# avabag01-ai/spectrogram-midi

Hardware: AMD Instinct MI355X
Metric: audio-seconds transcribed/sec (44.1 kHz, n_fft=2048) (higher is better)
Workload: dtype f64

## Files before the change

### spectrogram-midi_amd/csrc/aegis_handle.hip

```cpp
#include "aegis_internal.h"
#include "effects.h"

#include <chrono>
#include <cmath>
#include <cstdio>
#include <cstdlib>
#include <new>
#include <stdexcept>
#include <thread>

using namespace aegis;

static std::string g_create_error;

int aegis::grow_buf(aegis_handle *h, std::vector<DevBuf *> &owner, DevBuf &b, size_t bytes) {
    if (h->fail_allocs > 0) {
        --h->fail_allocs;
        h->err = "hipMalloc(" + std::to_string(bytes) + " bytes): out of memory (test hook)";
        return AEGIS_ERR_NOMEM;
    }
    if (b.p) {
        HIPCHK(h, hipDeviceSynchronize());
        HIPCHK(h, hipFree(b.p));
        b.p = nullptr; b.cap = 0;
    }
    if (!b.listed) { owner.push_back(&b); b.listed = true; }
    const size_t want = bytes + bytes / 8 + 256;
    hipError_t e = hipMalloc(&b.p, want);
    if (e != hipSuccess) {
        b.p = nullptr;
        h->err = "hipMalloc(" + std::to_string(want) + " bytes): " + hipGetErrorString(e);
        return AEGIS_ERR_NOMEM;
    }
    b.cap = want;
    return AEGIS_OK;
}

void aegis::free_bufs(std::vector<DevBuf *> &owner) noexcept {
    for (DevBuf *b : owner) {
        if (b->p) (void)hipFree(b->p);
        *b = DevBuf{};
    }
    owner.clear();
}

int aegis::new_event(aegis_handle *h, hipEvent_t *e, unsigned flags) {
    HIPCHK(h, hipEventCreateWithFlags(e, flags));
    h->owned_events.push_back(*e);
    return AEGIS_OK;
}

static int create_events(aegis_handle *h) {
    int rc = new_event(h, &h->copy_event, hipEventDisableTiming);
    h->sync_events.assign(8, nullptr);
    for (hipEvent_t &e : h->sync_events) if (rc == AEGIS_OK) rc = new_event(h, &e, hipEventDisableTiming);
    for (hipEvent_t &e : h->split_ev) if (rc == AEGIS_OK) rc = new_event(h, &e, hipEventDefault);
    for (hipEvent_t &e : h->hyb_ev) if (rc == AEGIS_OK) rc = new_event(h, &e, hipEventDisableTiming);
    for (hipEvent_t &e : h->fin_ev) if (rc == AEGIS_OK) rc = new_event(h, &e, hipEventDisableTiming);
    return rc;
}

template <typename T>
static int upload_table(aegis_handle *h, const std::vector<T> &v, const T **dst) {
    void *d = nullptr;
    const size_t bytes = std::max<size_t>(v.size() * sizeof(T), 16);
    HIPCHK(h, hipMalloc(&d, bytes));
    h->table_allocs.push_back(d);
    if (!v.empty()) HIPCHK(h, hipMemcpy(d, v.data(), v.size() * sizeof(T), hipMemcpyHostToDevice));
    *dst = static_cast<const T *>(d);
    return AEGIS_OK;
}

void aegis::begin_event(aegis_handle *h, const char *name, hipStream_t s) {
    if (!h->profiling) return;
    hipEvent_t a, b;
    if (hipEventCreate(&a) != hipSuccess || hipEventCreate(&b) != hipSuccess) return;
    (void)hipEventRecord(a, s);
    h->events.push_back({name, {a, b}});
}
void aegis::end_event(aegis_handle *h, hipStream_t s) {
    if (!h->profiling || h->events.empty()) return;
    (void)hipEventRecord(h->events.back().second.second, s);
}
void aegis::drop_events(aegis_handle *h) noexcept {
    for (auto &ev : h->events) { (void)hipEventDestroy(ev.second.first); (void)hipEventDestroy(ev.second.second); }
    h->events.clear();
}
void aegis::collect_events(aegis_handle *h) {
    h->last_ms.clear();
    h->last_count.clear();
    double total = 0;
    for (auto &ev : h->events) {
        float ms = 0;
        if (hipEventElapsedTime(&ms, ev.second.first, ev.second.second) == hipSuccess) {
            h->last_ms[ev.first] += ms;
            h->last_count[ev.first] += 1;
            total += ms;
        }
    }
    drop_events(h);
    h->last_ms["total"] = total;
}

int aegis::abi_fail(aegis_handle *h) noexcept {
    int code = AEGIS_ERR_DEVICE;
    const char *msg = "unknown C++ exception";
    std::string what;
    try { throw; }
    catch (const std::bad_alloc &) { code = AEGIS_ERR_NOMEM; msg = "out of host memory"; }
    catch (const std::length_error &) { code = AEGIS_ERR_NOMEM; msg = "request too large for a host container"; }
    catch (const std::exception &e) { try { what = e.what(); msg = what.c_str(); } catch (...) {} }
    catch (...) {}
    try { (h ? h->err : g_create_error) = msg; } catch (...) {}
    return code;
}

static const PassPlan *last_pass(const aegis_handle *h) { return h->plan.passes.empty() ? nullptr : &h->plan.passes.back(); }
static int last_work(const aegis_handle *h) { return h->plan.passes.empty() ? 0 : (int)((h->plan.passes.size() - 1) & 1); }

extern "C" {

int aegis_abi_version(void) { return AEGIS_ABI_VERSION; }

const char *aegis_last_error(const aegis_handle *h) { return h ? h->err.c_str() : g_create_error.c_str(); }

int aegis_create(const aegis_config *cfg, aegis_handle **out) {
    aegis_handle *h = nullptr;
    try {
    if (!out) { g_create_error = "out == NULL"; return AEGIS_ERR_INVALID; }
    *out = nullptr;
    aegis_config c{};
    if (cfg) c = *cfg;
    if (c.sample_rate == 0) c.sample_rate = 44100;
    if (c.hop_length == 0) c.hop_length = 512;
    if (c.n_fft == 0) c.n_fft = 2048;
    if (c.n_mels == 0) c.n_mels = 128;
    if (!(c.fmin > 0)) c.fmin = 82.4068892282175;
    if (!(c.fmax > 0)) c.fmax = 1046.5022612023945;
    const bool auto_pass = c.max_frames_per_pass <= 0;
    if (auto_pass) c.max_frames_per_pass = (int64_t)1 << 21;

    h = new (std::nothrow) aegis_handle();
    if (!h) { g_create_error = "out of host memory"; return AEGIS_ERR_NOMEM; }
    const std::string terr = h->tab.build(c.sample_rate, c.hop_length, c.n_fft, c.n_mels, c.fmin, c.fmax);
    if (!terr.empty()) { g_create_error = terr; delete h; return AEGIS_ERR_INVALID; }
    if (!h->tab.set_pyin_init(c.pyin_init)) { g_create_error = "pyin_init must be AEGIS_PYIN_INIT_UNVOICED (0) or AEGIS_PYIN_INIT_UNIFORM (1)"; delete h; return AEGIS_ERR_INVALID; }
    h->device = c.device;
    h->max_frames_per_pass = c.max_frames_per_pass;
    h->knobs.read_env();
    h->persist.on = h->knobs.persistent_wanted;

    h->lag_stride = (h->tab.max_period + 1 + 7) & ~7;
// ... 104 lines not shown
            bool busy = false;
            for (hipStream_t q : all) if (q && hipStreamQuery(q) == hipErrorNotReady) busy = true;
            if (!busy) break;
            if (std::chrono::steady_clock::now() - t0 > std::chrono::seconds(10)) {
                std::fprintf(stderr, "libaegis_hip: aegis_destroy: work still running on the handle's streams after 10 s; its device memory and streams are leaked\n");
                (void)hipGetLastError();
                delete h;
                return;
            }
            std::this_thread::sleep_for(std::chrono::milliseconds(1));
        }
        (void)hipGetLastError();
    }
    T("device sync");
    (void)hipDeviceSynchronize();
    for (auto &ss : h->split)
        for (hipStream_t q : {ss.frame_a, ss.frame_b, ss.viterbi})
            if (q) { T("destroy masked stream"); (void)hipStreamDestroy(q); }
    T("sync stream"); if (h->stream) (void)hipStreamSynchronize(h->stream);
    T("sync stream2"); if (h->stream2) (void)hipStreamSynchronize(h->stream2);
    T("sync stream3"); if (h->stream3) (void)hipStreamSynchronize(h->stream3);
    T("sync stream4"); if (h->stream4) (void)hipStreamSynchronize(h->stream4);
    T("events");
    drop_events(h);
    for (hipEvent_t e : h->owned_events) (void)hipEventDestroy(e);
    T("free tables");
    for (void *p : h->table_allocs) (void)hipFree(p);
    for (auto &cb : h->cqt_banks) if (cb.bank.dev) (void)hipFree(cb.bank.dev);
    h->cqt_banks.clear();
    T("free workspaces and staging");
    free_bufs(h->bufs);
    T("destroy streams");
    for (hipStream_t q : {h->stream, h->stream2, h->stream3, h->stream4}) if (q) (void)hipStreamDestroy(q);
    T("done");
    delete h;
}

extern "C" {

int64_t aegis_frames_for(const aegis_handle *h, int64_t n_samples) {
    try {
    if (!h || n_samples < 0) return AEGIS_ERR_INVALID;
    return 1 + n_samples / h->tab.hop;
    } catch (...) { return abi_fail(const_cast<aegis_handle *>(h)); }
}

int aegis_set_profiling(aegis_handle *h, int32_t on) {
    try {
    if (!h) return AEGIS_ERR_INVALID;
    h->profiling = on != 0;
    return AEGIS_OK;
    } catch (...) { return abi_fail(h); }
}

int aegis_last_kernel_launches(const aegis_handle *h, const char *name) {
    if (!h || !name) return -1;
    auto it = h->last_count.find(name);
    return it == h->last_count.end() ? 0 : it->second;
}

double aegis_last_kernel_ms(const aegis_handle *h, const char *name) {
    if (!h || !name) return -1.0;
    auto it = h->last_ms.find(name);
    return it == h->last_ms.end() ? -1.0 : it->second;
}

int aegis_set_table(aegis_handle *h, const char *name, const double *data, int64_t count) {
    try {
    if (!h || !name || !data) return AEGIS_ERR_INVALID;
    Tables &t = h->tab;
    const std::string n(name);
    struct Slot { std::vector<double> *host; const double *dev; };
    auto slot = [&](const std::string &nm) -> Slot {
        if (nm == "beta_probs") return {&t.beta_probs, h->dt.beta_probs};
        if (nm == "beta_cumsum") return {&t.beta_cumsum, h->dt.beta_cumsum};
        if (nm == "beta_suffix") return {&t.beta_suffix, h->dt.beta_suffix};
        if (nm == "boltz_fact") return {&t.boltz_fact, h->dt.boltz_fact};
        if (nm == "boltz_exp") return {&t.boltz_exp, h->dt.boltz_exp};
        if (nm == "freqs") return {&t.freqs, h->dt.freqs};
        return {nullptr, nullptr};
    };
    auto push = [&](const std::string &nm) -> int {
        Slot s = slot(nm);
        if (h->device < 0) return AEGIS_OK;
        HIPCHK(h, hipSetDevice(h->device));
        HIPCHK(h, hipStreamSynchronize(h->stream));
        HIPCHK(h, hipMemcpy(const_cast<double *>(s.dev), s.host->data(), s.host->size() * 8, hipMemcpyHostToDevice));
        return AEGIS_OK;
    };
    Slot s = slot(n);
    if (!s.host || n == "beta_cumsum" || n == "beta_suffix") { h->err = "unknown or derived table: " + n; return AEGIS_ERR_INVALID; }
    if (count != (int64_t)s.host->size()) {
        h->err = "table " + n + " needs " + std::to_string(s.host->size()) + " entries";
        return AEGIS_ERR_INVALID;
    }
    std::copy(data, data + count, s.host->begin());
    int rc = push(n);
    if (rc != AEGIS_OK) return rc;
    if (n == "beta_probs") {
        for (int k = 0; k <= kNThresholds; ++k) t.beta_cumsum[k] = np_pairwise_sum(t.beta_probs.data(), k);
        t.beta_suffix.assign(kNThresholds + 1, 0.0);
        for (int k = kNThresholds - 1; k >= 0; --k) t.beta_suffix[k] = t.beta_suffix[k + 1] + t.beta_probs[k];
        if ((rc = push("beta_cumsum")) != AEGIS_OK) return rc;
        if ((rc = push("beta_suffix")) != AEGIS_OK) return rc;
    }
    return AEGIS_OK;
    } catch (...) { return abi_fail(h); }
}

int64_t aegis_get_param(const aegis_handle *h, const char *name) {
    try {
    if (!h || !name) return AEGIS_ERR_INVALID;
    const Tables &t = h->tab;
    const std::string n(name);
    if (n == "min_period") return t.min_period;
    if (n == "max_period") return t.max_period;
    if (n == "n_lags") return t.n_lags;
    if (n == "n_pitch_bins") return t.n_bins;
    if (n == "transition_width") return t.width;
    if (n == "n_trans_classes") return t.n_cls;
    if (n == "max_frames_per_pass") return h->max_frames_per_pass;
    if (n == "lag_stride") return h->lag_stride;
    if (n == "yin_stride") return h->yin_stride;
    if (n == "obs_stride") return h->obs_stride;
    const PassPlan *lp = last_pass(h);
    if (n == "last_frames") return lp ? lp->fp : 0;
    if (n == "last_passes") return (int64_t)h->plan.passes.size();
    if (n == "last_split_segments") { int64_t v = 0; for (const PassPlan &q : h->plan.passes) v += q.tsplit ? q.n_seg : 0; return v; }
    if (n == "split_passes") return h->tsplit.stats[0];
    if (n == "split_segments") return h->tsplit.stats[1];
    if (n == "split_flagged_clips") return h->tsplit.stats[2];
    if (n == "split_unlocked_clips") return h->tsplit.stats[3];
    if (n == "split_rounds") return h->tsplit.last_carried_steps;
    if (n == "split_viterbi_us") return (int64_t)(h->tsplit.last_viterbi_ms * 1e3);
    if (n == "split_cooldown") return h->tsplit.cooldown;
    if (n == "last_chunks") return lp ? lp->nk() : 0;
    if (n == "last_dense") return lp ? lp->dense : 0;
    if (n == "last_proportional") return lp ? lp->proportional : 0;
    if (n == "last_balanced") return lp ? lp->balanced : 0;
    if (n == "last_hybrid_step") return lp ? lp->hyb_S : 0;
    if (n == "last_persistent") return lp ? lp->persistent : 0;
    if (n == "pyin_init") return t.pyin_init;
    if (n == "cqt_bank_builds") return h->cqt_bank_builds;
    if (n == "cqt_banks") return (int64_t)h->cqt_banks.size();
    if (n == "cqt_bank_cap") return h->cqt_bank_cap;
    if (n == "cqt_bank_bytes") return h->cqt_bank_bytes;
    if (n == "cqt_bank_build_us") return h->cqt_bank_build_us;
    if (n == "cmnd_in_frame") return cmnd_in_frame(h);
    if (n == "troughs_in_frame") return troughs_in_frame(h);
    if (n == "frame_fpw") return frame_batch_fpw(t.max_period);
    if (n == "obs_waves") { PassParams q = base_params(t); q.n_sel = 4096; return pyin_obs_waves(q); }
    if (n == "viterbi_kernel") { const int k = viterbi_kernel_choice(base_params(t), rule_tables(h)); return k < 0 ? AEGIS_ERR_UNSUPPORTED : k; }
    if (n == "split_applies") return viterbi_split_applies(base_params(t), rule_tables(h)) ? 1 : 0;
    if (n == "fx_tile") return kFxRevTile;
    if (n == "fx_chunk") return kFxChunk;
    if (n == "fx_max_taps") return kFxMaxTaps;
    return AEGIS_ERR_INVALID;
    } catch (...) { return abi_fail(const_cast<aegis_handle *>(h)); }
}

int64_t aegis_get_table(const aegis_handle *h, const char *name, void *dst, int64_t cap) {
    try {
    if (!h || !name) return AEGIS_ERR_INVALID;
    const Tables &t = h->tab;
    const std::string n(name);
    const void *src = nullptr;
    int64_t count = 0;
    size_t esz = 8;
    auto setd = [&](const std::vector<double> &v) { src = v.data(); count = (int64_t)v.size(); esz = 8; };
    if (n == "hann") setd(t.hann);
    else if (n == "thresholds") setd(t.thresholds);
    else if (n == "beta_probs") setd(t.beta_probs);
    else if (n == "beta_cumsum") setd(t.beta_cumsum);
    else if (n == "beta_suffix") setd(t.beta_suffix);
    else if (n == "boltz_fact") setd(t.boltz_fact);
    else if (n == "boltz_exp") setd(t.boltz_exp);
    else if (n == "log_trans_band") setd(t.log_trans_band);
    else if (n == "log_trans_pack") setd(t.log_trans_pack);
    else if (n == "freqs") setd(t.freqs);
    else if (n == "bin_edges") setd(t.bin_edges);
    else if (n == "twiddle") setd(t.twiddle);
    else if (n == "tuning_edges") setd(h->tuning_edges);
    else if (n == "mel_dense") { src = t.mel_dense.data(); count = (int64_t)t.mel_dense.size(); esz = 4; }
    else return AEGIS_ERR_INVALID;
    if (dst && cap > 0) std::memcpy(dst, src, (size_t)std::min(count, cap) * esz);
    return count;
    } catch (...) { return abi_fail(const_cast<aegis_handle *>(h)); }
}

int64_t aegis_debug_plan(aegis_handle *h, const int64_t *n_samples, int32_t n_clips, int32_t entry, int32_t sync,
                         int32_t n_cus, int64_t *dst, int64_t cap) {
    try {
    if (!h || n_clips < 0 || (n_clips > 0 && !n_samples) || cap < 0 || (cap > 0 && !dst)) return AEGIS_ERR_INVALID;
    std::lock_guard<std::mutex> lock(h->mu);
    std::vector<int64_t> off((size_t)n_clips + 1, 0);
    for (int i = 0; i < n_clips; ++i) {
        if (n_samples[i] < 0 || 1 + n_samples[i] / h->tab.hop > h->max_frames_per_pass) { h->err = "bad clip " + std::to_string(i); return AEGIS_ERR_INVALID; }
        off[i + 1] = off[i] + n_samples[i];
    }
    const int kind = entry & 3;
    const PlanKnobs &kn = h->knobs;
    PlanInput in = plan_input(h, off.data(), n_clips, AEGIS_STAGE_ALL, kind == AEGIS_PLAN_HOST_FED, kind == AEGIS_PLAN_CALLER_STREAM,
                              sync, n_cus, [&kn, n_cus](int n) { return masked_streams_fit(kn, n_cus, n); });
    if (entry & AEGIS_PLAN_COOLING) in.cooling = split_allowed(in) && kn.split_seglen < 0;
    if (entry & AEGIS_PLAN_NO_PERSIST) in.persistent = false;
    const CallPlan c = plan_call(in);
    std::vector<int64_t> v{(int64_t)c.passes.size()};
    for (const PassPlan &m : c.passes) {
        const int64_t flags = m.tsplit * AEGIS_PLAN_F_SPLIT | m.split_auto * AEGIS_PLAN_F_SPLIT_AUTO | m.want_hybrid * AEGIS_PLAN_F_WANT_HYBRID |
                              m.hybrid * AEGIS_PLAN_F_HYBRID | m.hyb_part * AEGIS_PLAN_F_HYBRID_PART | m.balanced * AEGIS_PLAN_F_BALANCED |
                              m.may_persist * AEGIS_PLAN_F_MAY_PERSIST | m.persistent * AEGIS_PLAN_F_PERSISTENT | m.dense * AEGIS_PLAN_F_DENSE |
                              m.proportional * AEGIS_PLAN_F_PROPORTIONAL | m.two_fs * AEGIS_PLAN_F_TWO_FRAME_STREAMS | m.use_fb * AEGIS_PLAN_F_FRAME_B;
        const int64_t lanes = (int64_t)m.fa | (int64_t)m.fb << 4 | (int64_t)m.sv << 8 | (int64_t)m.sd << 12 | (int64_t)m.sa << 16;
        uint64_t hash = 1469598103934665603ull;
        auto mix = [&hash](const void *p, size_t n) {
            for (size_t i = 0; i < n; ++i) { hash ^= static_cast<const unsigned char *>(p)[i]; hash *= 1099511628211ull; }
        };
        auto table = [&mix](const auto &t) { const uint64_t n = t.size(); mix(&n, 8); mix(t.data(), n * sizeof(t[0])); };
        table(m.seg32); table(m.seg64); table(m.sel_off); table(m.clip_tb);
        for (int64_t x : {(int64_t)m.nc(), m.fp, m.maxF, flags, m.seglen, m.hyb_S, (int64_t)m.n_seg, (int64_t)m.n_lock, (int64_t)m.nk(),
                          (int64_t)m.ramp_k, lanes, (int64_t)hash}) v.push_back(x);
        v.insert(v.end(), m.cb.begin(), m.cb.end());
    }
    if (cap > 0) std::memcpy(dst, v.data(), (size_t)std::min<int64_t>(cap, (int64_t)v.size()) * 8);
    return (int64_t)v.size();
    } catch (...) { return abi_fail(h); }
}

struct Counter { const char *name; int count; hipError_t (*fetch)(long long *); bool always_sync; };
static const Counter kCounters[] = {
    {"obs_cycles", 16, obs_debug_fetch, false},
    {"frame_cycles", 24, frame_debug_fetch, false},
    {"split_verify", 16, [](long long *v) { return viterbi_verify_fetch(v, true); }, false},
    {"viterbi_cycles", 128, [](long long *v) { return viterbi_debug_fetch(v, true); }, false},
    {"viterbi_spans", 272, viterbi_span_fetch, false},
    {"cqt_cycles", 16, cqt_debug_fetch, true},
};

int64_t aegis_debug_fetch(aegis_handle *h, const char *name, void *dst, int64_t cap) {
    try {
    if (!h || !name) return AEGIS_ERR_INVALID;
    const std::string n(name);
    if (n == "throw_bad_alloc") throw std::bad_alloc();
    if (n == "throw_length_error") throw std::length_error("test hook");
    if (n == "throw_runtime_error") throw std::runtime_error("test hook: runtime_error");
    if (n == "throw_int") throw 42;
    if (n == "fail_allocs") { h->fail_allocs = (int)std::max<int64_t>(0, cap); return 0; }
    for (const Counter &c : kCounters) {
        if (n != c.name) continue;
        if (h->device < 0) return AEGIS_ERR_INVALID;
        if (c.always_sync || (dst && cap > 0)) {
            long long v[272];
            HIPCHK(h, hipSetDevice(h->device));
            HIPCHK(h, hipDeviceSynchronize());
            HIPCHK(h, c.fetch(v));
            if (dst && cap > 0) std::memcpy(dst, v, (size_t)std::min<int64_t>(cap, c.count) * 8);
        }
        return c.count;
    }
    const PassPlan *lp = last_pass(h);
    const int64_t F = lp ? lp->fp : 0;
    const int last_pass_segments = lp && lp->tsplit ? lp->n_seg : 0;
    const void *src = nullptr;
    int64_t count = 0;
    size_t esz = 8;
    const aegis_handle::Work &lw = h->work[last_work(h)];
    if (n == "dfn") { src = lw.dfn.p; count = F * h->lag_stride; }
    else if (n == "yin") { src = lw.yin.p; count = F * h->yin_stride; }
    else if (n == "logobs") {
        count = F * h->obs_stride;
        if (h->device < 0 || !lw.logobs.p || !lw.obs_seg.p) { h->err = "stage was not run"; return AEGIS_ERR_INVALID; }
        if (dst && cap > 0) {
            HIPCHK(h, hipSetDevice(h->device));
            HIPCHK(h, hipStreamSynchronize(h->stream));
            std::vector<double> rows((size_t)count);
            std::vector<int32_t> seg((size_t)F);
            HIPCHK(h, hipMemcpy(rows.data(), lw.logobs.p, (size_t)count * 8, hipMemcpyDeviceToHost));
            HIPCHK(h, hipMemcpy(seg.data(), lw.obs_seg.p, (size_t)F * 4, hipMemcpyDeviceToHost));
            const double log_tiny = h->tab.log_tiny;
            for (int64_t f = 0; f < F; ++f)
                for (int b = 0; b < h->obs_stride; ++b)
                    if (!(seg[(size_t)f] & (0x40000000 | (1 << (b >> 6))))) rows[(size_t)(f * h->obs_stride + b)] = log_tiny;
            std::memcpy(dst, rows.data(), (size_t)std::min(count, cap) * 8);
        }
        return count;
    }
    else if (n == "logunv") { src = lw.logunv.p; count = F; }
    else if (n == "obs_seg") { src = lw.obs_seg.p; count = F; esz = 4; }
    else if (n == "states") { src = lw.states.p; count = F; esz = 4; }
    else if (n == "melpow") { src = lw.melpow.p; count = F * h->tab.n_mels; esz = 4; }
    else if (n == "rake_raw") { src = lw.rake_raw.p; count = F; esz = 1; }
    else if (n == "tuning_peak_off") {
        const std::vector<int64_t> &po = h->tn_last_peak_off;
        if (dst && cap > 0) std::memcpy(dst, po.data(), (size_t)std::min<int64_t>(cap, (int64_t)po.size()) * 8);
        return (int64_t)po.size();
    }
    else if (n == "tuning_pitch" || n == "tuning_mag" || n == "tuning_median") {
        if (h->tn_last_peak_off.empty()) return 0;
        if (n == "tuning_median") { src = h->tn_median.p; count = (int64_t)h->tn_last_peak_off.size() - 1; }
        else { src = n == "tuning_pitch" ? h->tn_pitch.p : h->tn_mag.p; count = h->tn_last_peak_off.back(); }
        esz = 4;
    }
    else if (n == "persistent_fallbacks") {
        if (dst && cap > 0) *static_cast<int64_t *>(dst) = h->persist.fallbacks;
        return 1;
    }
// ... 172 lines not shown
```

### spectrogram-midi_amd/csrc/viterbi.hip

```cpp
#include <functional>
#include "kernels.h"
#include "pass_geometry.h"
#include "wave_ops.h"

#include <algorithm>
#include <cfloat>
#include <cmath>
#include <cstdlib>
#include <cstring>

namespace aegis {

__global__ __launch_bounds__(1024) void viterbi_kernel(PassParams p, DevTables tb, int lt_in_lds) {
    extern __shared__ __align__(16) unsigned char smem_raw[];
    const int B = p.n_bins, S = 2 * B, H = p.half_width, W = p.width, NC = p.n_cls;
    const int SP = (S + 63) & ~63;
    constexpr int C = kViterbiChunk;
    double *val = reinterpret_cast<double *>(smem_raw);
    double *rv = val + 2 * SP;
    int *ri = reinterpret_cast<int *>(rv + 32);
    uint16_t *ring = reinterpret_cast<uint16_t *>(ri + 32);
    double *ltl = reinterpret_cast<double *>(smem_raw + ((2 * SP + 32) * 8 + 32 * 4 + C * S * 2 + 15) / 16 * 16);

    const int tid = threadIdx.x, nthr = blockDim.x, lane = tid & 63, wid = tid >> 6, nw = nthr >> 6;
    if (lt_in_lds)
        for (int i = tid; i < 4 * NC * W; i += nthr) ltl[i] = tb.lt_band[i];
    const double *lt = lt_in_lds ? ltl : tb.lt_band;

    const int c = p.order[blockIdx.x];
    const int64_t f0 = p.frame_off[c];
    const int T = (int)(p.frame_off[c + 1] - f0);
    const int os = p.obs_stride;
    const double *__restrict__ lobs = p.logobs + f0 * os;
    const double *__restrict__ lunv = p.logunv + f0;
    const int32_t *__restrict__ oseg = p.obs_seg + f0;
    auto voiced_obs = [&](int t, int b) {
        const int sg = oseg[t];
        return (sg & (0x40000000 | (1 << (b >> 6)))) ? lobs[(int64_t)t * os + b] : p.log_tiny;
    };
    uint16_t *__restrict__ ptr = p.ptr + f0 * S;
    const int64_t ch0 = p.chunk_off[c];
    uint16_t *__restrict__ cmap = p.cmap + ch0 * S;
    int32_t *__restrict__ bnd = p.bnd + ch0;
    int32_t *__restrict__ states = p.states + f0;
    const int nch = (T - 1 + C - 1) / C;

    const int j = tid;
    const bool act = j < S;
    const int v2 = (j >= B) ? 1 : 0;
    const int b2 = j - v2 * B;
    const int dlo = max(0, H - b2);
    const int dhi = min(W - 1, B - 1 - b2 + H);

    const int64_t vt_begin = p.clip_t0 ? p.clip_t0[c] : geo_vt_begin(p), vt_end = p.clip_t0 ? p.clip_t1[c] : geo_vt_end(p);
    if (p.ctl && p.ctl->n_sel == 0) return;
    const int t_lo = (int)(vt_begin > 1 ? vt_begin : 1);
    const int t_hi = (int)(vt_end < T ? vt_end : T);
    if (vt_begin >= T && vt_begin != 0) return;
    double *__restrict__ vst = p.vstate + (int64_t)c * S;
    double myv = -INFINITY;
    if (act) {
        if (vt_begin == 0) {
            const double lp = v2 ? lunv[0] : voiced_obs(0, b2);
            myv = lp + (v2 ? p.log_pinit_u : p.log_pinit_v);
        } else {
            myv = vst[j];
        }
        val[j] = myv;
    }
    int par = 0;
    double G;
    int kg;
    auto block_argmax = [&](double v, int ix) {
#pragma unroll
        for (int o = 32; o >= 1; o >>= 1) {
            const double ov = __shfl_down(v, o);
            const int oi = __shfl_down(ix, o);
            if (ov > v || (ov == v && oi < ix)) { v = ov; ix = oi; }
        }
        if (lane == 0) { rv[par * 16 + wid] = v; ri[par * 16 + wid] = ix; }
        __syncthreads();
        G = rv[par * 16]; kg = ri[par * 16];
        for (int w = 1; w < nw; ++w) {
            const double ov = rv[par * 16 + w];
            const int oi = ri[par * 16 + w];
            if (ov > G || (ov == G && oi < kg)) { G = ov; kg = oi; }
        }
        par ^= 1;
    };
    block_argmax(myv, act ? j : 0x7fffffff);
    if (p.live_states != nullptr && tid == 0 && vt_begin == 0) p.live_states[f0] = kg;

    double *cur = val, *nxt = val + SP;
    for (int t = t_lo; t < t_hi; ++t) {
        double lp = 0.0;
        if (act) lp = v2 ? lunv[t] : voiced_obs(t, b2);
        double best = -INFINITY;
        int bi = 0;
        if (act) {
#pragma unroll
            for (int v = 0; v < 2; ++v) {
                const double *cv = cur + v * B;
                const double *ltv = lt + (size_t)(v * 2 + v2) * NC * W;
                for (int d = dlo; d <= dhi; ++d) {
                    const int b = b2 + d - H;
                    const int cl = b < H ? b : (b > B - 1 - H ? b - (B - 1 - 2 * H) : H);
                    const double cand = cv[b] + ltv[cl * W + (W - 1 - d)];
                    if (cand > best) { best = cand; bi = v * B + b; }
                }
            }
            const int bg = kg >= B ? kg - B : kg;
            const int dist = bg > b2 ? bg - b2 : b2 - bg;
            if (dist > H) {
                const double cand = G + p.log_tiny;
                if (cand > best || (cand == best && kg < bi)) { best = cand; bi = kg; }
            }
            myv = lp + best;
            nxt[j] = myv;
            ring[((t - 1) % C) * S + j] = (uint16_t)bi;
            ptr[(int64_t)t * S + j] = (uint16_t)bi;
        }
        block_argmax(myv, act ? j : 0x7fffffff);
        if (p.live_states != nullptr && tid == 0) p.live_states[f0 + t] = kg;
        double *tmp = cur; cur = nxt; nxt = tmp;
        if (t % C == 0 || t == T - 1) {
            const int cc = (t - 1) / C;
            if (act) {
                int s = j;
                for (int tt = t; tt > cc * C; --tt)
                    s = tt >= t_lo ? ring[((tt - 1) % C) * S + s] : ptr[(int64_t)tt * S + s];
                cmap[(int64_t)cc * S + j] = (uint16_t)s;
            }
            __syncthreads();
        }
    }

    if (t_hi < T) {
        if (act) vst[j] = myv;
        return;
    }
    if (tid == 0) {
        int s = kg;
        for (int cc = nch - 1; cc >= 0; --cc) { bnd[cc] = s; s = cmap[(int64_t)cc * S + s]; }
        states[0] = s;
    }
    __threadfence();
    __syncthreads();
    for (int cc = tid; cc < nch; cc += nthr) {
        const int te = min((cc + 1) * C, T - 1);
        int s = bnd[cc];
        states[te] = s;
        for (int tt = te; tt > cc * C + 1; --tt) { s = ptr[(int64_t)tt * S + s]; states[tt - 1] = s; }
    }
}

template <int CTRL, int ROW_MASK>
__device__ __forceinline__ double dpp_fmax(double v) {
    const int lo = __double2loint(v), hi = __double2hiint(v);
    const int lo2 = __builtin_amdgcn_update_dpp(lo, lo, CTRL, ROW_MASK, 0xf, false);
    const int hi2 = __builtin_amdgcn_update_dpp(hi, hi, CTRL, ROW_MASK, 0xf, false);
    return fmax(v, __hiloint2double(hi2, lo2));
}
__device__ __forceinline__ double row16_prefix_max(double v) {
    v = dpp_fmax<0x111, 0xf>(v);
    v = dpp_fmax<0x112, 0xf>(v);
    v = dpp_fmax<0x114, 0xf>(v);
    v = dpp_fmax<0x118, 0xf>(v);
    return v;
}
__device__ __forceinline__ double wave_max_neg(double v, unsigned long long &at) {
    const unsigned hi = (unsigned)__double2hiint(v), lo = (unsigned)__double2loint(v);
    const unsigned mh = wave_umin(hi);
    const bool top = hi == mh;
    const unsigned long long tb = __ballot(top);
    unsigned ml;
    if ((tb & (tb - 1)) == 0) {
        ml = (unsigned)__builtin_amdgcn_readlane((int)lo, (int)__ffsll((long long)tb) - 1);
        at = tb;
    } else {
        ml = wave_umin(top ? lo : 0xffffffffu);
        at = __ballot(top && lo == ml);
    }
    return __hiloint2double((int)mh, (int)ml);
}
__device__ __forceinline__ double wave_min_bound_neg(double v, bool take) {
    const unsigned hi = take ? (unsigned)__double2hiint(v) : 0u;
    return __hiloint2double((int)wave_umax(hi), -1);
}
__device__ __forceinline__ double min_f64_raw(double a, double b) {
    double r;
    asm("v_min_f64 %0, %1, %2" : "=v"(r) : "v"(a), "v"(b));
    return r;
}
__device__ __forceinline__ double read_lane_f64(double v, int l) {
    return __hiloint2double(__builtin_amdgcn_readlane(__double2hiint(v), l),
                            __builtin_amdgcn_readlane(__double2loint(v), l));
}

template <int H> __host__ __device__ constexpr int pk_lo_start(int e) { return 1 + e * (H + 1) + e * (e - 1) / 2; }
template <int H> __host__ __device__ constexpr int pk_int_start() { return 1 + H * (H + 1) + H * (H - 1) / 2; }
template <int H> __host__ __device__ constexpr int pk_hi_start(int e) { return pk_int_start<H>() + (2 * H + 1) + 2 * H * e - e * (e - 1) / 2; }
template <int H> __host__ __device__ constexpr int pk_size() { return 3 * H * H + 3 * H + 2; }
__host__ __device__ constexpr bool band_table_packed(int) { return true; }

template <int H>
struct BandLT {
    double v[4][2 * H + 1];
    double lmax[4];
    double lmax_all;
};

#if defined(AEGIS_ABLATE) && (AEGIS_ABLATE & 64)
__device__ long long g_vit_dbg[16 * 8];
#define VIT_TICK(k) { const long long now__ = clock64(); tacc[k] += now__ - tlast; tlast = now__; }
#else
#define VIT_TICK(k)
#endif

#if defined(AEGIS_ABLATE) && (AEGIS_ABLATE & 512)
__device__ unsigned long long g_vit_span[272];
#endif
#ifndef AEGIS_VIT_GATE
#define AEGIS_VIT_GATE 1
#endif
#ifndef AEGIS_VIT_GROUP50
#define AEGIS_VIT_GROUP50 0
#endif
#ifndef AEGIS_VIT_GROUP
#define AEGIS_VIT_GROUP 7
#endif
#define VIT_SPLIT 0
template <int H, bool LT_LDS>
__global__ __launch_bounds__(1024) void viterbi_band_kernel(PassParams p, DevTables tb, BandLT<H> blt) {
#include "viterbi_band.inc"
}
template <int H, bool LT_LDS>
__global__ __launch_bounds__(1024) __attribute__((amdgpu_waves_per_eu(5, 5))) void viterbi_band_dense_kernel(PassParams p, DevTables tb, BandLT<H> blt) {
#include "viterbi_band.inc"
}
#undef VIT_SPLIT
#define VIT_SPLIT 1
template <int H, bool LT_LDS>
__global__ __launch_bounds__(1024) void viterbi_band_split_kernel(PassParams p, DevTables tb, BandLT<H> blt) {
#include "viterbi_band.inc"
}
#undef VIT_SPLIT

__device__ __forceinline__ bool clip_selected(const PassParams &p, int c) {
    return p.clip_sel == 0 || ((p.clip_dirty[c] != 0) == (p.clip_sel == 2));
}
__global__ __launch_bounds__(1024) void viterbi_segmap_kernel(PassParams p) {
    constexpr int C = kViterbiChunk;
    const int sg = blockIdx.x, S = 2 * p.n_bins, j = threadIdx.x;
    if (j >= S || !clip_selected(p, p.seg_clip[sg])) return;
    const int T = p.seg_T[sg], st = p.seg_store[sg];
    const uint16_t *__restrict__ cmap = p.cmap + p.seg_ch0[sg] * S;
    int s = j;
    if (T - 1 > st)
        for (int cc = (T - 2) / C; cc >= st / C; --cc) {
            s = cmap[(int64_t)cc * S + s];
            if (s >= S) { s = 0; break; }
        }
    p.seg_map[(int64_t)sg * S + j] = (uint16_t)s;
}
__global__ __launch_bounds__(64) void viterbi_round_kernel(PassParams p, int round) {
    const int c = blockIdx.x * 64 + threadIdx.x;
    if (c >= p.n_clips) return;
    int k = -1;
    for (int sg = p.clip_seg0[c] + 1; sg < p.clip_seg0[c + 1]; ++sg)
        if (p.seg_lock[sg] == -1) { k = sg; break; }
    p.clip_first[c] = k;
    if (round == 0) p.clip_dirty[c] = k >= 0 ? 1 : 0;
    if (k >= 0) { p.seg_lock[k] = -2; atomicMax(p.tube_count + 1, (uint32_t)(round + 1)); }
}
__global__ __launch_bounds__(1024) void viterbi_seg0_fill_kernel(PassParams p) {
    __shared__ double wmax[16];
    __shared__ int wkg[16];
    const int c = blockIdx.x, S = 2 * p.n_bins, j = threadIdx.x, lane = j & 63, w = j >> 6;
    const int a = p.clip_seg0[c], b = p.clip_seg0[c + 1];
    if (b - a < 2) return;
    const int64_t f = p.frame_off[c] + p.hybrid_step;
    const double v = j < S ? p.vstate[(int64_t)c * S + j] : -INFINITY;
    if (j < S) { p.seg_col[(int64_t)a * S + j] = v; p.colhist[f * (int64_t)S + j] = v; }
    double m = v;
#pragma unroll
    for (int o = 32; o >= 1; o >>= 1) m = fmax(m, __shfl_xor(m, o));
    const unsigned long long at = __ballot(j < S && v == m);
    if (lane == 0) { wmax[w] = m; wkg[w] = at ? w * 64 + (int)__ffsll((long long)at) - 1 : 0x7fffffff; }
    __syncthreads();
    if (j == 0) {
        double G = -INFINITY;
        int kg = 0x7fffffff;
        for (int k = 0; k < (int)(blockDim.x >> 6); ++k)
            if (wmax[k] > G || (wmax[k] == G && wkg[k] < kg)) { G = wmax[k]; kg = wkg[k]; }
        p.colG[f] = G; p.colkg[f] = kg; p.seg_kg[a] = kg;
    }
}
__global__ __launch_bounds__(64) void viterbi_stitch_kernel(PassParams p) {
    const int c = blockIdx.x * 64 + threadIdx.x;
    if (c >= p.n_clips) return;
    const int S = 2 * p.n_bins, a = p.clip_seg0[c], b = p.clip_seg0[c + 1];
    if (p.split_hybrid && b - a < 2) return;
    if (!clip_selected(p, c)) return;
    bool bad = false;
    for (int k = a + 1; k < b; ++k) bad |= p.seg_lock[k] == -1;
    int e = p.seg_kg[b - 1];
    for (int k = b - 1; k >= a; --k) { p.seg_end[k] = e; e = p.seg_map[(int64_t)k * S + e]; }
    p.states[p.frame_off[c]] = e;
    if (bad) atomicOr(&p.clip_flag[c], 1u);
}
__global__ __launch_bounds__(256) void viterbi_segtrace_kernel(PassParams p) {
    constexpr int C = kViterbiChunk;
    const int sg = blockIdx.x, S = 2 * p.n_bins, tid = threadIdx.x;
    const int T = p.seg_T[sg], st = p.seg_store[sg];
    if (T - 1 <= st || !clip_selected(p, p.seg_clip[sg])) return;
    const int64_t f0 = p.seg_f0[sg], ch0 = p.seg_ch0[sg];
    const uint16_t *__restrict__ cmap = p.cmap + ch0 * S;
    const uint16_t *__restrict__ ptr = p.ptr + f0 * S;
    int32_t *__restrict__ bnd = p.bnd + ch0;
    int32_t *__restrict__ states = p.states + f0;
    const int cfirst = st / C, clast = (T - 2) / C;
    if (tid == 0) {
        int s = p.seg_end[sg];
        for (int cc = clast; cc >= cfirst; --cc) { bnd[cc] = s; s = cmap[(int64_t)cc * S + s]; }
    }
    __threadfence();
    __syncthreads();
    for (int cc = cfirst + tid; cc <= clast; cc += blockDim.x) {
        const int te = min((cc + 1) * C, T - 1);
        int s = bnd[cc];
        states[te] = s;
        for (int tt = te; tt > cc * C + 1; --tt) { s = ptr[(int64_t)tt * S + s]; states[tt - 1] = s; }
    }
}

constexpr int kTubeCap = 16, kTubeDepth = 48;
constexpr int kTubeRec = 4 + (kTubeDepth + 1) * (1 + kTubeCap) + 2;
constexpr int kRailAt = kTubeRec - 2, kRailLen = kTubeRec - 1;
__device__ unsigned long long g_verify_dbg[16];

__device__ __forceinline__ double split_bound(const PassParams &p, int64_t fr, int64_t fc, int nsp) {
    const double g = fabs(p.colG[fr - 1]) + 1500.0;
    return 2.0 * (nsp * (1e-7 + 1e-13 * g) + 4.5e-16 * (double)(fr - fc) * g);
}
__device__ __forceinline__ double split_lt(const PassParams &p, const DevTables &tb, int si, int sj) {
    const int B = p.n_bins, H = p.half_width, W = p.width;
    const int v = si >= B ? 1 : 0, v2 = sj >= B ? 1 : 0, bs = si - v * B, b2 = sj - v2 * B;
    const int cl = bs < H ? bs : (bs > B - 1 - H ? bs - (B - 1 - 2 * H) : H);
    return tb.lt_band[((size_t)(v * 2 + v2) * p.n_cls + cl) * W + (b2 - bs + H)];
}
__device__ __forceinline__ double split_obs(const PassParams &p, int j, int64_t fr) {
    const int B = p.n_bins;
    if (j >= B) return p.logunv[fr];
    return (p.obs_seg[fr] & (0x40000000 | (1 << (j >> 6)))) ? p.logobs[fr * (int64_t)p.obs_stride + j] : p.log_tiny;
}

__global__ __launch_bounds__(256) void viterbi_verify_kernel(PassParams p, DevTables tb) {
    constexpr int CAP = kTubeCap;
    __shared__ int sets[4][2][CAP];
    const int lane = threadIdx.x & 63, w = threadIdx.x >> 6;
    const int B = p.n_bins, S = 2 * B, H = p.half_width, W = p.width, NC = p.n_cls;
    const int64_t idx = (int64_t)blockIdx.x * 4 + w;
    if (idx >= p.vf_total) return;
    int lo = 0, hi = p.n_clips;
    while (hi - lo > 1) { const int mid = (lo + hi) >> 1; if (p.vf_off[mid] <= idx) lo = mid; else hi = mid; }
    const int c = lo;
    const int a = p.clip_seg0[c], b = p.clip_seg0[c + 1];
    if (b - a < 2 || !clip_selected(p, c)) return;
    const int64_t fc = p.frame_off[c];
    const int64_t fx = p.seg_f0[a + 1] + p.seg_store[a + 1];
    const int64_t f = fx + 1 + (idx - p.vf_off[c]);
    if (f >= p.frame_off[c + 1]) return;
    const int Tc = (int)(p.frame_off[c + 1] - fc), nsp = b - a;
    int why = 0;
    auto near_preds = [&](int j, int64_t fr, double thr, int *dst, int &n) {
        const int v2 = j >= B ? 1 : 0, b2 = j - v2 * B;
        const double *__restrict__ col = p.colhist + (fr - 1) * (int64_t)S;
        const double G = p.colG[fr - 1];
        const int kg = p.colkg[fr - 1];
        double cand[4];
        double best = -INFINITY;
#pragma unroll
        for (int v = 0; v < 2; ++v)
#pragma unroll
            for (int r = 0; r < 2; ++r) {
                const int d = lane + 64 * r, bs = b2 + d - H;
                double cv = -INFINITY;
                if (d < W && bs >= 0 && bs < B) {
                    const int cl = bs < H ? bs : (bs > B - 1 - H ? bs - (B - 1 - 2 * H) : H);
                    cv = col[v * B + bs] + tb.lt_band[((size_t)(v * 2 + v2) * NC + cl) * W + (W - 1 - d)];
                }
                cand[v * 2 + r] = cv;
                best = fmax(best, cv);
            }
        const int bg = kg >= B ? kg - B : kg;
        const bool oob = (bg > b2 ? bg - b2 : b2 - bg) > H;
#pragma unroll
        for (int o = 32; o >= 1; o >>= 1) best = fmax(best, __shfl_xor(best, o));
        if (oob && G + p.log_tiny >= fmax(best, G + p.log_tiny) - thr) {
            best = fmax(best, G + p.log_tiny);
            int cnt = 0;
            for (int j0 = 0; j0 < S; j0 += 64) cnt += __popcll(__ballot(j0 + lane < S && col[j0 + lane] >= G - thr));
            if (cnt > 1) why = why ? why : 9;
            else {
                bool have = false;
                for (int q = 0; q < n; ++q) have |= dst[q] == kg;
                if (!have) { if (n < CAP) dst[n++] = kg; else why = why ? why : 3; }
            }
        }
#pragma unroll
        for (int v = 0; v < 2; ++v)
#pragma unroll
            for (int r = 0; r < 2; ++r) {
                unsigned long long m = __ballot(cand[v * 2 + r] >= best - thr);
                while (m) {
                    const int l = (int)__ffsll((long long)m) - 1;
                    m &= m - 1;
                    const int sidx = v * B + b2 + l + 64 * r - H;
                    bool have = false;
                    for (int q = 0; q < n; ++q) have |= dst[q] == sidx;
                    if (!have) { if (n < CAP) dst[n++] = sidx; else why = why ? why : 3; }
                }
            }
    };
    int *cur = sets[w][0], *nxt = sets[w][1];
    cur[0] = p.states[f];
    int n = 1;
    if (f == fc + Tc - 1) {
        const double *__restrict__ col = p.colhist + f * (int64_t)S;
        const double thr = split_bound(p, f + 1, fc, nsp), G = p.colG[f];
        n = 0;
        for (int j0 = 0; j0 < S; j0 += 64) {
            unsigned long long m = __ballot(j0 + lane < S && col[j0 + lane] >= G - thr);
            while (m) { const int l = (int)__ffsll((long long)m) - 1; m &= m - 1; if (n < CAP) cur[n++] = j0 + l; else why = 3; }
        }
    } else {
        int m1 = 0, w0 = why;
        near_preds(p.states[f + 1], f + 1, split_bound(p, f + 1, fc, nsp), nxt, m1);
        if (why == w0 && m1 > 1) return;
        why = w0;
        if (f + 1 == fc + Tc - 1) {
            const double *__restrict__ col = p.colhist + (f + 1) * (int64_t)S;
            const double thr = split_bound(p, f + 2, fc, nsp), G = p.colG[f + 1];
            int cnt = 0;
            for (int j0 = 0; j0 < S; j0 += 64) cnt += __popcll(__ballot(j0 + lane < S && col[j0 + lane] >= G - thr));
            if (cnt > 1) return;
        }
    }
    auto rail_scan = [&](const int *mem, int nm, int64_t ftop) -> int {
        int L = 0;
        const int64_t maxL = ftop - fx;
        while (L < maxL) {
            const int64_t fk = ftop - L - lane;
            bool ok = fk > fx;
            if (ok) {
                const double thr = split_bound(p, fk, fc, nsp);
                const double *__restrict__ col = p.colhist + (fk - 1) * (int64_t)S;
                const double G = p.colG[fk - 1];
                const int kg = p.colkg[fk - 1], bg = kg >= B ? kg - B : kg;
                for (int q = 0; q < nm && ok; ++q) {
                    const int b2 = mem[q] - B;
                    const int blo = b2 - H > 0 ? b2 - H : 0, bhi = b2 + H < B - 1 ? b2 + H : B - 1;
                    const int clj = b2 < H ? b2 : (b2 > B - 1 - H ? b2 - (B - 1 - 2 * H) : H);
                    const double self = col[B + b2] + tb.lt_band[((size_t)3 * NC + clj) * W + H];
                    double other = -INFINITY;
                    for (int v = 0; v < 2; ++v) {
                        const double *__restrict__ cv = col + v * B;
                        const double *__restrict__ ltv = tb.lt_band + (size_t)(v * 2 + 1) * NC * W;
#pragma unroll 8
                        for (int bs = blo; bs <= bhi; ++bs) {
                            const int cl = bs < H ? bs : (bs > B - 1 - H ? bs - (B - 1 - 2 * H) : H);
                            const double x = cv[bs] + ltv[cl * W + (H + b2 - bs)];
                            other = fmax(other, (v == 1 && bs == b2) ? -INFINITY : x);
                        }
                    }
                    ok = other < self - thr && !((bg > b2 ? bg - b2 : b2 - bg) > H && G + p.log_tiny >= self - thr);
                }
            }
// ... 481 lines not shown
```

### spectrogram-midi_amd/csrc/viterbi_band.inc

```
    constexpr int W = 2 * H + 1;
    constexpr int C = kViterbiChunk;
    extern __shared__ __align__(16) unsigned char smem_raw[];
    const int B = p.n_bins, S = 2 * B, NC = p.n_cls;
    const int BP = (B + 63) & ~63;
    const int PADB = (B + 2 * H + 64 + 7) & ~7;
    const int PB = 2 * PADB + 4 * H;
    double *val = reinterpret_cast<double *>(smem_raw);
    double *rv = val + 2 * PB;
    unsigned long long *omask = reinterpret_cast<unsigned long long *>(rv + 64);
    int *ri = reinterpret_cast<int *>(omask + 32);
    uint16_t *ring = reinterpret_cast<uint16_t *>(ri + 32);
    double *ltl = reinterpret_cast<double *>(
        smem_raw + (((size_t)(4 * PADB + 8 * H + 96) * 8 + 32 * 4 + (size_t)2 * S * 2 + 15) / 16) * 16);
    constexpr int NP = pk_size<H>();
    constexpr int KG = H + 63, NGATE = 3 * H + 64;
    double *gate = ltl + (band_table_packed(H) ? 2 * NP : 4 * NC * W);
    constexpr bool PK = LT_LDS && band_table_packed(H);

    const int tid = threadIdx.x, nthr = blockDim.x, lane = tid & 63, wid = tid >> 6, nw = nthr >> 6;
    const int vp = __builtin_amdgcn_readfirstlane(tid >= BP ? 1 : 0);
    const int b2 = tid - vp * BP;
    const bool act = b2 < B;
    const int b2c = act ? b2 : 0;
    const int j = vp * B + b2c;
// ... 417 lines not shown
                    const int rowbase = !PK ? (lo_e ? bo : (hi_e ? bo - (B - 1 - 2 * H) : H)) * W
                                            : lo_e ? pk_lo_start<H>(bo) - (H - bo)
                                                   : (hi_e ? pk_hi_start<H>(bo - (B - H)) : pk_int_start<H>());
                    const int dd = b2c - bo + H;
                    const int off = (act && (unsigned)dd < (unsigned)W) ? rowbase + dd : kSentinel;
                    const double cand = vo + lt_e0[off];
                    if (cand > best) src = bo;
                    best = fmax(best, cand);
                }
            }
        } else {
            double besta = -INFINITY, bestb = -INFINITY;
            int codea = 0, codeb = 0;
#pragma unroll
            for (int d = 0; d < HALF; ++d) {
                const double cand = vi0[d] + lti0[W - 1 - d];
                if (cand > besta) codea = d;
                besta = fmax(besta, cand);
                if (HALF + d < W) {
                    const double candb = vi0[HALF + d] + lti0[W - 1 - HALF - d];
                    if (candb > bestb) codeb = HALF + d;
                    bestb = fmax(bestb, candb);
                }
            }
            if (bestb > besta) { besta = bestb; codea = codeb; }
            best = besta;
            src = b2c + codea - H;
#if !(defined(AEGIS_ABLATE) && (AEGIS_ABLATE & 1))
            if (wave_low) {
                double eb = -INFINITY;
                int ec = 0;
#pragma unroll
                for (int e = 0; e < H; ++e) {
                    const double cand = edge_lo(ve0, lt_e0, e);
                    if (cand > eb) ec = e;
                    eb = fmax(eb, cand);
                }
                if (eb >= best) { best = eb; src = ec; }
            }
            if (wave_high) {
                double eb = -INFINITY;
                int ec = 0;
#pragma unroll
                for (int e = 0; e < H; ++e) {
                    const double cand = edge_hi(ve0, lt_e0, e);
                    if (cand > eb) ec = e;
                    eb = fmax(eb, cand);
                }
                if (eb > best) { best = eb; src = B - H + ec; }
            }
#endif
        }
        VIT_TICK(1)
        bi = src;
        if (best1 > best) { best = best1; bi = B + src1; }
        {
            const int bg = kg >= B ? kg - B : kg;
            if ((unsigned)(b2c + (H - bg)) > (unsigned)(2 * H)) {
                const double cand = G + p.log_tiny;
                if (cand > best || (cand == best && kg < bi)) { best = cand; bi = kg; }
            }
        }
        }
        const double sum = lp + best;
        myv = (act && !skip) ? sum : -INFINITY;
        observed = act && !vp && !skip && lp != p.log_tiny;
        n_skip += skip ? 1 : 0;
#if VIT_SPLIT
        const bool st = t > store_from;
        const bool lockchk = lockon && (t % C == 0);
        if (lockchk) {
            const double old = act ? p.colhist[(f0 + t) * (int64_t)S + j] : -INFINITY;
            const bool fin_n = myv > -INFINITY, fin_o = old > -INFINITY;
            const bool bad = act && (fin_n != fin_o);
            const bool use = act && fin_n && fin_o;
            double dmin = use ? myv - old : INFINITY, dmax = use ? myv - old : -INFINITY;
#pragma unroll
            for (int o = 32; o >= 1; o >>= 1) { dmin = fmin(dmin, __shfl_xor(dmin, o)); dmax = fmax(dmax, __shfl_xor(dmax, o)); }
            const bool anybad = __ballot(bad) != 0ull;
            if (lane == 0) { lk[wid] = dmin; lk[16 + wid] = dmax; lk[32 + wid] = anybad ? 1.0 : 0.0; }
        }
#if !(defined(AEGIS_SPLIT_ABLATE) && (AEGIS_SPLIT_ABLATE & 1))
        if (act && st) p.colhist[(f0 + t) * (int64_t)S + j] = myv;
#endif
#else
        constexpr bool st = true;
#endif
        if (skip) {
            if (act) store_value(cur ^ 1, -INFINITY);
        } else if (act) {
            store_value(cur ^ 1, myv);
            if (st) ptr[(int64_t)t * S + j] = (uint16_t)bi;
            const uint16_t o = ((t - 1) % C == 0) ? (uint16_t)bi : org[cur * S + bi];
            org[(cur ^ 1) * S + j] = o;
            if (st && (t % C == 0 || t == T - 1)) cmap[(int64_t)((t - 1) / C) * S + j] = o;
        }
        VIT_TICK(2)
        end_of_step(myv, observed, cur ^ 1);
        VIT_TICK(3)
        if (p.live_states != nullptr && tid == 0) p.live_states[f0 + t] = kg;
#if VIT_SPLIT
#if !(defined(AEGIS_SPLIT_ABLATE) && (AEGIS_SPLIT_ABLATE & 2))
        if (tid == 0 && st) { p.colG[f0 + t] = G; p.colkg[f0 + t] = kg; }
#endif
        if (lockchk) {
            double dmin = lane < nw ? lk[lane] : INFINITY, dmax = lane < nw ? lk[16 + lane] : -INFINITY;
            const bool bad = lane < nw && lk[32 + lane] != 0.0;
#pragma unroll
            for (int o = 8; o >= 1; o >>= 1) { dmin = fmin(dmin, __shfl_xor(dmin, o)); dmax = fmax(dmax, __shfl_xor(dmax, o)); }
            dmin = __shfl(dmin, 0); dmax = __shfl(dmax, 0);
            const double sigma = 1e-7 + 1e-13 * fabs(G);
            if (__ballot(bad) == 0ull && dmax - dmin <= sigma) { locked_at = t; ph ^= 1; ++t; break; }
        }
#endif
        ph ^= 1;
        VIT_TICK(4)
    }
#if VIT_SPLIT
    if (locked_at >= 0) break;
#endif
    }
#if defined(AEGIS_ABLATE) && (AEGIS_ABLATE & 64)
    if (blockIdx.x == 0 && lane == 0) {
        for (int k = 0; k < 6; ++k) atomicAdd((unsigned long long *)&g_vit_dbg[wid * 8 + k], (unsigned long long)tacc[k]);
        atomicAdd((unsigned long long *)&g_vit_dbg[wid * 8 + 7], (unsigned long long)(t_hi - t_lo));
    }
#endif

    if (p.vstats != nullptr && lane == 0 && t_hi > t_lo) {
        atomicAdd(&p.vstats[0], (unsigned long long)(t_hi - t_lo));
        atomicAdd(&p.vstats[1], (unsigned long long)n_list);
        atomicAdd(&p.vstats[2], (unsigned long long)n_skip);
    }
#if VIT_SPLIT
    if (lockon) {
        if (tid == 0) p.seg_lock[c] = locked_at;
        if (locked_at < 0) {
            if (act) p.seg_col2[(int64_t)c * S + j] = myv;
            if (c == p.clip_seg0[ci + 1] - 1) {
                if (act) p.seg_col[(int64_t)c * S + j] = myv;
                if (tid == 0) p.seg_kg[c] = kg;
            }
        }
    } else {
        if (act) p.seg_col[(int64_t)c * S + j] = myv;
        if (tid == 0) { p.seg_kg[c] = kg; if (exact_seg) p.seg_lock[c] = 0; }
    }
    return;
#else
    if (t_hi < T) {
        if (act) vst[j] = myv;
        return;
    }
    if (tid == 0) {
        int s = kg;
        for (int cc = nch - 1; cc >= 0; --cc) { bnd[cc] = s; s = cmap[(int64_t)cc * S + s]; }
        states[0] = s;
    }
    __threadfence();
    __syncthreads();
    for (int cc = tid; cc < nch; cc += nthr) {
        const int te = min((cc + 1) * C, T - 1);
        int s = bnd[cc];
        states[te] = s;
        for (int tt = te; tt > cc * C + 1; --tt) { s = ptr[(int64_t)tt * S + s]; states[tt - 1] = s; }
    }
#endif
```

Measured before the change: 316,500.

## Parallelize Viterbi chunk-boundary backtrace across threads using group composition

Replaces the single-thread serial walk over chunk maps in the Viterbi backtrace with a three-phase parallel scheme. Chunks are split into groups, and for every possible end state each thread composes the group's maps into a table in reused shared memory. One thread then chains the group ends, and each group's boundaries are filled in parallel. This targets the serial tail of the backtrace, at the cost of about S times more cmap reads and extra barriers and shared memory. The dense band variant keeps the serial path.

```diff
diff --git a/spectrogram-midi_amd/csrc/aegis_handle.hip b/spectrogram-midi_amd/csrc/aegis_handle.hip
--- a/spectrogram-midi_amd/csrc/aegis_handle.hip
+++ b/spectrogram-midi_amd/csrc/aegis_handle.hip
@@ -1,3 +1,4 @@
+#include "backtrace.h"
 #include "aegis_internal.h"
 #include "effects.h"
 
@@ -408,6 +409,7 @@
     if (n == "obs_waves") { PassParams q = base_params(t); q.n_sel = 4096; return pyin_obs_waves(q); }
     if (n == "viterbi_kernel") { const int k = viterbi_kernel_choice(base_params(t), rule_tables(h)); return k < 0 ? AEGIS_ERR_UNSUPPORTED : k; }
     if (n == "split_applies") return viterbi_split_applies(base_params(t), rule_tables(h)) ? 1 : 0;
+    if (n == "backtrace_groups") return kBacktraceGroups;
     if (n == "fx_tile") return kFxRevTile;
     if (n == "fx_chunk") return kFxChunk;
     if (n == "fx_max_taps") return kFxMaxTaps;
diff --git a/spectrogram-midi_amd/csrc/backtrace.h b/spectrogram-midi_amd/csrc/backtrace.h
--- /dev/null
+++ b/spectrogram-midi_amd/csrc/backtrace.h
@@ -0,0 +1,96 @@
+#pragma once
+#include <cstdint>
+
+#if defined(__HIPCC__)
+#include <hip/hip_runtime.h>
+#define AEGIS_BT_HD __host__ __device__ __forceinline__
+#else
+#define AEGIS_BT_HD inline
+#endif
+
+namespace aegis {
+
+#ifndef AEGIS_BT_GROUPS
+#define AEGIS_BT_GROUPS 16
+#endif
+constexpr int kBacktraceGroups = AEGIS_BT_GROUPS;
+#ifndef AEGIS_BT_BATCH
+#define AEGIS_BT_BATCH 8
+#endif
+constexpr int kBtBatch = AEGIS_BT_BATCH;
+
+struct BtPlan {
+    int ng;
+    int gl;
+};
+AEGIS_BT_HD BtPlan bt_plan(int c_lo, int c_hi, int S, int e_cap) {
+    BtPlan pl = {0, 0};
+    const int n = c_hi - c_lo + 1;
+    int gmax = e_cap / (S + 1);
+    if (gmax > kBacktraceGroups) gmax = kBacktraceGroups;
+    if (n < 2 * kBacktraceGroups || gmax < 2) return pl;
+    pl.gl = (n + gmax - 1) / gmax;
+    pl.ng = (n + pl.gl - 1) / pl.gl;
+    return pl;
+}
+
+AEGIS_BT_HD int bt_serial(const uint16_t *__restrict__ cmap, int32_t *__restrict__ bnd, int S, int c_lo, int c_hi, int s) {
+    for (int cc = c_hi; cc >= c_lo; --cc) { bnd[cc] = s; s = cmap[(int64_t)cc * S + s]; }
+    return s;
+}
+
+AEGIS_BT_HD void bt_phase_a(const BtPlan pl, const uint16_t *__restrict__ cmap, int S, int c_lo, int c_hi,
+                            uint16_t *E, int tid, int nthr) {
+    for (int e = tid; e < S; e += nthr)
+        for (int g0 = 0; g0 < pl.ng; g0 += kBtBatch) {
+            int s[kBtBatch];
+#pragma unroll
+            for (int k = 0; k < kBtBatch; ++k) s[k] = e;
+            for (int j = pl.gl - 1; j >= 0; --j) {
+#pragma unroll
+                for (int k = 0; k < kBtBatch; ++k) {
+                    const int cc = c_lo + (g0 + k) * pl.gl + j;
+                    if (g0 + k < pl.ng && cc <= c_hi) {
+                        const int v = cmap[(int64_t)cc * S + s[k]];
+                        s[k] = v < S ? v : 0;
+                    }
+                }
+            }
+#pragma unroll
+            for (int k = 0; k < kBtBatch; ++k)
+                if (g0 + k < pl.ng) E[(g0 + k) * S + e] = (uint16_t)s[k];
+        }
+}
+
+AEGIS_BT_HD void bt_phase_b(const BtPlan pl, int S, uint16_t *E, int e) {
+    uint16_t *ends = E + pl.ng * S;
+    for (int g = pl.ng - 1; g >= 0; --g) { ends[g] = (uint16_t)e; e = E[g * S + e]; }
+}
+
+AEGIS_BT_HD int bt_phase_c(const BtPlan pl, const uint16_t *__restrict__ cmap, int32_t *__restrict__ bnd, int S,
+                           int c_lo, int c_hi, const uint16_t *E, int g) {
+    const int bot = c_lo + g * pl.gl;
+    const int top = bot + pl.gl - 1 < c_hi ? bot + pl.gl - 1 : c_hi;
+    return bt_serial(cmap, bnd, S, bot, top, E[pl.ng * S + g]);
+}
+
+#if defined(__HIPCC__)
+__device__ __forceinline__ int bt_block(const uint16_t *__restrict__ cmap, int32_t *__restrict__ bnd, int S, int c_lo, int c_hi,
+                                        int e, uint16_t *E, int e_cap) {
+    const int tid = threadIdx.x, nthr = blockDim.x;
+#if defined(AEGIS_ABLATE) && (AEGIS_ABLATE & 2048)
+    for (int cc = c_lo + tid; cc <= c_hi; cc += nthr) bnd[cc] = S / 2;
+    return S / 2;
+#endif
+    const BtPlan pl = bt_plan(c_lo, c_hi, S, e_cap);
+    if (pl.ng == 0) return tid == 0 ? bt_serial(cmap, bnd, S, c_lo, c_hi, e) : 0;
+    __syncthreads();
+    bt_phase_a(pl, cmap, S, c_lo, c_hi, E, tid, nthr);
+    __syncthreads();
+    if (tid == 0) bt_phase_b(pl, S, E, e);
+    __syncthreads();
+    return tid < pl.ng ? bt_phase_c(pl, cmap, bnd, S, c_lo, c_hi, E, tid) : 0;
+}
+#endif
+
+}
diff --git a/spectrogram-midi_amd/csrc/viterbi.hip b/spectrogram-midi_amd/csrc/viterbi.hip
--- a/spectrogram-midi_amd/csrc/viterbi.hip
+++ b/spectrogram-midi_amd/csrc/viterbi.hip
@@ -2,6 +2,7 @@
 #include "kernels.h"
 #include "pass_geometry.h"
 #include "wave_ops.h"
+#include "backtrace.h"
 
 #include <algorithm>
 #include <cfloat>
@@ -139,10 +140,11 @@
         if (act) vst[j] = myv;
         return;
     }
-    if (tid == 0) {
-        int s = kg;
-        for (int cc = nch - 1; cc >= 0; --cc) { bnd[cc] = s; s = cmap[(int64_t)cc * S + s]; }
-        states[0] = s;
+    {
+        const int cap_lt = lt_in_lds ? 16 * NC * W : 0, cap_val = 8 * SP;
+        uint16_t *E = reinterpret_cast<uint16_t *>(cap_lt > cap_val ? ltl : val);
+        const int s = bt_block(cmap, bnd, S, 0, nch - 1, kg, E, max(cap_lt, cap_val));
+        if (tid == 0) states[0] = s;
     }
     __threadfence();
     __syncthreads();
@@ -230,14 +232,18 @@
 #define AEGIS_VIT_GROUP 7
 #endif
 #define VIT_SPLIT 0
+#define VIT_DENSE 0
 template <int H, bool LT_LDS>
 __global__ __launch_bounds__(1024) void viterbi_band_kernel(PassParams p, DevTables tb, BandLT<H> blt) {
 #include "viterbi_band.inc"
 }
+#undef VIT_DENSE
+#define VIT_DENSE 1
 template <int H, bool LT_LDS>
 __global__ __launch_bounds__(1024) __attribute__((amdgpu_waves_per_eu(5, 5))) void viterbi_band_dense_kernel(PassParams p, DevTables tb, BandLT<H> blt) {
 #include "viterbi_band.inc"
 }
+#undef VIT_DENSE
 #undef VIT_SPLIT
 #define VIT_SPLIT 1
 template <int H, bool LT_LDS>
@@ -309,8 +315,10 @@
     p.states[p.frame_off[c]] = e;
     if (bad) atomicOr(&p.clip_flag[c], 1u);
 }
+constexpr int kSegtraceBtCap = 16 * (1024 + 1);
 __global__ __launch_bounds__(256) void viterbi_segtrace_kernel(PassParams p) {
     constexpr int C = kViterbiChunk;
+    __shared__ uint16_t bt_e[kSegtraceBtCap];
     const int sg = blockIdx.x, S = 2 * p.n_bins, tid = threadIdx.x;
     const int T = p.seg_T[sg], st = p.seg_store[sg];
     if (T - 1 <= st || !clip_selected(p, p.seg_clip[sg])) return;
@@ -320,10 +328,7 @@
     int32_t *__restrict__ bnd = p.bnd + ch0;
     int32_t *__restrict__ states = p.states + f0;
     const int cfirst = st / C, clast = (T - 2) / C;
-    if (tid == 0) {
-        int s = p.seg_end[sg];
-        for (int cc = clast; cc >= cfirst; --cc) { bnd[cc] = s; s = cmap[(int64_t)cc * S + s]; }
-    }
+    bt_block(cmap, bnd, S, cfirst, clast, p.seg_end[sg], bt_e, kSegtraceBtCap);
     __threadfence();
     __syncthreads();
     for (int cc = cfirst + tid; cc <= clast; cc += blockDim.x) {
diff --git a/spectrogram-midi_amd/csrc/viterbi_band.inc b/spectrogram-midi_amd/csrc/viterbi_band.inc
--- a/spectrogram-midi_amd/csrc/viterbi_band.inc
+++ b/spectrogram-midi_amd/csrc/viterbi_band.inc
@@ -593,11 +593,16 @@
         if (act) vst[j] = myv;
         return;
     }
-    if (tid == 0) {
-        int s = kg;
-        for (int cc = nch - 1; cc >= 0; --cc) { bnd[cc] = s; s = cmap[(int64_t)cc * S + s]; }
-        states[0] = s;
-    }
+#if VIT_DENSE
+    if (tid == 0) states[0] = bt_serial(cmap, bnd, S, 0, nch - 1, kg);
+#else
+    {
+        uint16_t *E = reinterpret_cast<uint16_t *>(LT_LDS ? ltl : val);
+        const int e_cap = LT_LDS ? 4 * ((PK ? 2 * NP : 4 * NC * W) + NGATE) : 8 * PB;
+        const int s = bt_block(cmap, bnd, S, 0, nch - 1, kg, E, e_cap);
+        if (tid == 0) states[0] = s;
+    }
+#endif
     __threadfence();
     __syncthreads();
     for (int cc = tid; cc < nch; cc += nthr) {
```

Result: no change. 316,500, median of 2 (+0.0%).
